# fcogidi/X3D-tf

Hardware: AMD Instinct MI355X
Metric: clips/sec (fwd+bwd) X3D-M 16x224^2; depthwise HBM GB/s (higher is better)
Workload: dtype bf16

## Files before the change

### x3d-tf_amd/csrc/pw_bwd_wst.hip

```cpp
#include <stdlib.h>

#include "pw_gemm_ws.h"

struct PwBwdWstArgs {
  const void* g; const void* yraw; const float* coef;
  const void* wp; int wp_rows;
  void* dx;
  const void* braw; const float* b_ss; const float* egate; double* nc_sums;
  float* dw;
  int N, Co, Ci;
  long long P;
  int tiles_per_block;
  BnBwdFold fold;
  float* slab;
  int hot;
  int noflush;
};

#define BW_YRP 40

template <typename H, int NW, int KS, int CT>
__global__ __launch_bounds__(512, 2) void pw_bwd_wst_kernel(const PwBwdWstArgs a) {
  typedef typename HV<H>::x8 hx8;
  extern __shared__ __attribute__((aligned(16))) unsigned char smem_raw[];
  typedef H T;
  constexpr int BN = 32, OP = WS_OP, NT = 512, Kp = KS * 16, WP = Kp + 8, CoP = CT * 32, YRP = BW_YRP;
  static_assert(CoP >= Kp, "the row-read copy covers every staged dY row");
  constexpr int NSV = (Kp * 4 + NT - 1) / NT;
  H* Yt = (H*)smem_raw;
  H* Yr = (H*)(smem_raw + (size_t)2 * Kp * 64);
  H* Xh = (H*)(smem_raw + (size_t)2 * Kp * 64 + (size_t)2 * CoP * YRP * 2);
  float* Cs = (float*)(smem_raw + (size_t)2 * Kp * 64 + (size_t)2 * CoP * YRP * 2 + (size_t)NW * 32 * YRP * 2);
  float* Os = Cs + Kp * 4;
  const int tid = threadIdx.x, lane = tid & 63, wid = tid >> 6;
  const int r = lane & 31, half = lane >> 5;
  const int mt = (a.Ci + 31) >> 5;
  const int tiles_per_n = (int)((a.P + BN - 1) / BN);
  const int total_tiles = tiles_per_n * a.N;
  const int tile_begin = blockIdx.x * a.tiles_per_block;
  const int tile_end = min(tile_begin + a.tiles_per_block, total_tiles);
  if (tile_begin >= tile_end) return;
  float* myOs = Os + wid * 32 * OP;
  const int rb = blockIdx.y * NW + wid;
  const bool mw = wid < NW && rb < mt;

  {
    hx8 z;
#pragma unroll
    for (int e = 0; e < 8; e++) z[e] = (H)0.f;
    for (int i = tid; i < 2 * CoP * YRP / 8; i += NT) ((hx8*)Yr)[i] = z;
    for (int k = tid; k < Kp; k += NT) {
      f32x4 c = {0.f, 0.f, 0.f, 0.f};
      if (k < a.Co) {
        float cA_, cB_, cC_;
        bn_bwd_coef_load(a.coef, a.fold, k, blockIdx.x == 0 && blockIdx.y == 0, cA_, cB_, cC_);
        c[0] = cA_; c[1] = cB_; c[2] = cC_;
      }
      *(f32x4*)&Cs[k * 4] = c;
    }
  }

  hx8 A[KS];
  if (mw) {
    const H* wt = (const H*)a.wp + (long long)a.wp_rows * WP + ((long long)rb * KS * 64 + lane) * 8;
#pragma unroll
    for (int ks = 0; ks < KS; ks++) A[ks] = *(const hx8*)(wt + ks * 512);
  } else {
#pragma unroll
    for (int ks = 0; ks < KS; ks++)
#pragma unroll
      for (int e = 0; e < 8; e++) A[ks][e] = (H)0.f;
  }

  hx8 g0[NSV], y0[NSV], g1[NSV], y1[NSV];
  auto issue_loads = [&](int tile_, hx8 (&gr)[NSV], hx8 (&yr)[NSV]) {
    const int tile = a.hot ? tile_begin : min(tile_, tile_end - 1);
    const int n = tile / tiles_per_n;
    const long long p0 = (long long)(tile - n * tiles_per_n) * BN;
#pragma unroll
    for (int i = 0; i < NSV; i++) {
      const int v = tid + i * NT;
      const int k = v >> 2;
      const long long p = p0 + (v & 3) * 8;
      const bool ok = k < a.Co && p < a.P;
      const long long o = ok ? ((long long)n * a.Co + k) * a.P + p : 0;
      gr[i] = *(const hx8*)((const T*)a.g + o);
      yr[i] = *(const hx8*)((const T*)a.yraw + o);
    }
  };
  auto commit = [&](int tile, int buf, const hx8 (&gr)[NSV], const hx8 (&yr)[NSV]) {
    const int n = tile / tiles_per_n;
    const long long p0 = (long long)(tile - n * tiles_per_n) * BN;
#pragma unroll
    for (int i = 0; i < NSV; i++) {
      const int v = tid + i * NT;
      const int k = v >> 2;
      if (k >= Kp) continue;
      const bool ok = k < a.Co && p0 + (v & 3) * 8 < a.P;
      const f32x4 cf = *(const f32x4*)&Cs[k * 4];
      float val[8];
#pragma unroll
      for (int e = 0; e < 8; e++) val[e] = ok ? cf[0] * (float)gr[i][e] + cf[1] * (float)yr[i][e] + cf[2] : 0.f;
      hx8 hv;
#pragma unroll
      for (int e = 0; e < 8; e++) hv[e] = (H)val[e];
      *(hx8*)&Yt[(buf * Kp + k) * BN + (v & 3) * 8] = hv;
      *(hx8*)&Yr[(buf * CoP + k) * YRP + (v & 3) * 8] = hv;
    }
  };

  const int row = lane >> 1, c0 = 16 * (lane & 1);
  const int m = rb * 32 + row;
  const bool mrow = mw && m < a.Ci;
  hx8 eb0[2], eb1[2];
  float gl0, gl1;
  const float* gsrc = a.egate ? a.egate : a.b_ss;
  auto issue_braw = [&](int tile_, hx8 (&eb)[2], float& gl) {
    const int tile = a.hot ? tile_begin : min(tile_, tile_end - 1);
    const int n = tile / tiles_per_n;
    const long long p0 = (long long)(tile - n * tiles_per_n) * BN;
    gl = gsrc[(a.egate && mrow) ? (long long)n * a.Ci + m : 0];
#pragma unroll
    for (int hv = 0; hv < 2; hv++) {
      const long long p = p0 + c0 + 8 * hv;
      const long long o = (mrow && p < a.P) ? ((long long)n * a.Ci + m) * a.P + p : 0;
      eb[hv] = *(const hx8*)((const T*)a.braw + o);
    }
  };

  float st1 = 0.f, st2 = 0.f;
  auto flush_sums = [&](int n) {
    const float s1 = st1 + dpp_get<0xB1, 0xF>(st1), s2 = st2 + dpp_get<0xB1, 0xF>(st2);
    if (mrow && (lane & 1) == 0) {
      double* d = a.nc_sums + ((long long)n * a.Ci + m) * 2;
      atomic_add_d(d, (double)s1);
      atomic_add_d(d + 1, (double)s2);
    }
    st1 = 0.f;
    st2 = 0.f;
  };
  const float sb = mrow ? a.b_ss[m * 2] : 0.f, tb = mrow ? a.b_ss[m * 2 + 1] : 0.f;

  f32x16 acc_dw[CT];
#pragma unroll
  for (int s = 0; s < CT; s++)
#pragma unroll
    for (int e = 0; e < 16; e++) acc_dw[s][e] = 0.f;

  const int g16 = lane >> 4, q = (lane & 15) >> 2, pp = lane & 3;
  const int tr_off = (8 * (g16 >> 1) + q) * BN + 16 * (g16 & 1) + 4 * pp;
  typedef s16x4 __attribute__((address_space(3))) * lds_s16x4_ptr;

  int n_prev = tile_begin / tiles_per_n;
  issue_loads(tile_begin, g0, y0);
  issue_braw(tile_begin, eb0, gl0);
  __syncthreads();
  commit(tile_begin, 0, g0, y0);
  __syncthreads();
  issue_loads(tile_begin + 1, g1, y1);
  issue_loads(tile_begin + 2, g0, y0);

  typedef __attribute__((ext_vector_type(4))) unsigned int u32x4_;
  auto step = [&](int tile, int cur, hx8 (&gr)[NSV], hx8 (&yr)[NSV], hx8 (&eb)[2], float gl, hx8 (&ebn)[2], float& gln) {
    const int n = tile / tiles_per_n;
    const long long p0 = (long long)(tile - n * tiles_per_n) * BN;
    if (n != n_prev) flush_sums(n_prev);
    n_prev = n;
    issue_braw(tile + 1, ebn, gln);
    const float gt = (mrow && a.egate) ? gl : 1.0f;
    __amdgpu_buffer_rsrc_t dxr = __builtin_amdgcn_make_buffer_rsrc((T*)a.dx + (long long)n * a.Ci * a.P, 0,
                                                                   (int)((long long)a.Ci * a.P * 2), 0x00020000);

    f32x16 acc;
#pragma unroll
    for (int e = 0; e < 16; e++) acc[e] = 0.f;
    if (mw) {
      const H* xb = Yt + cur * (Kp * BN) + tr_off;
#pragma unroll
      for (int ks = 0; ks < KS; ks++) {
        const s16x4 b0 = __builtin_amdgcn_ds_read_tr16_b64_v4i16((lds_s16x4_ptr)(xb + ks * 16 * BN));
        const s16x4 b1 = __builtin_amdgcn_ds_read_tr16_b64_v4i16((lds_s16x4_ptr)(xb + (ks * 16 + 4) * BN));
        const s16x8 bs = {b0[0], b0[1], b0[2], b0[3], b1[0], b1[1], b1[2], b1[3]};
        acc = mfma16<H>(A[ks], __builtin_bit_cast(hx8, bs), acc);
      }
    }

    if (tile + 1 < tile_end) commit(tile + 1, cur ^ 1, gr, yr);

    if (mw) {
#pragma unroll
      for (int e = 0; e < 16; e++) myOs[((e & 3) + 8 * (e >> 2) + 4 * half) * OP + r] = acc[e];
#pragma unroll
      for (int hv = 0; hv < 2; hv++) {
        const long long p = p0 + c0 + 8 * hv;
        const bool ok = mrow && p < a.P;
        float val[8];
        {
          const f32x4 v0 = *(const f32x4*)&myOs[row * OP + c0 + 8 * hv], v1 = *(const f32x4*)&myOs[row * OP + c0 + 8 * hv + 4];
#pragma unroll
          for (int e = 0; e < 4; e++) { val[e] = v0[e]; val[4 + e] = v1[e]; }
        }
        hx8 xh;
        const SwishCoef sc_ = swish_coef(sb, tb, gt);
#pragma unroll
        for (int e = 0; e < 8; e++) {
          const float b = (float)eb[hv][e];
          float xs, d_;
          swish_bwd_(sc_, b, xs, d_);
          xh[e] = ok ? (H)xs : (H)0.f;
          const float dv = val[e] * d_;
          val[e] = dv;
          if (ok) { st1 += dv; st2 += dv * b; }
        }
        *(hx8*)&Xh[(wid * 32 + row) * YRP + c0 + 8 * hv] = xh;
        hx8 ov;
#pragma unroll
        for (int e = 0; e < 8; e++) ov[e] = (H)val[e];
        __builtin_amdgcn_raw_buffer_store_b128(__builtin_bit_cast(u32x4_, ov), dxr,
                                               ok ? (unsigned)(((long long)m * a.P + p) * 2) : 0x80000000u, 0, 0);
      }
      const H* yrow = Yr + (cur * CoP + r) * YRP + 8 * half;
      const H* xrow = Xh + (wid * 32 + r) * YRP + 8 * half;
#pragma unroll
      for (int ks = 0; ks < BN / 16; ks++) {
        const hx8 bf = *(const hx8*)(xrow + ks * 16);
#pragma unroll
        for (int s = 0; s < CT; s++) {
          const hx8 af = *(const hx8*)(yrow + s * 32 * YRP + ks * 16);
          acc_dw[s] = mfma16<H>(af, bf, acc_dw[s]);
        }
      }
    }
    __syncthreads();
    issue_loads(tile + 3, gr, yr);
  };
  for (int tile = tile_begin; tile < tile_end; tile += 2) {
    step(tile, 0, g1, y1, eb0, gl0, eb1, gl1);
    if (tile + 1 < tile_end) step(tile + 1, 1, g0, y0, eb1, gl1, eb0, gl0);
  }
  flush_sums(n_prev);

  if (mw && !a.noflush) {
    const int ci = rb * 32 + r;
    float* slab = a.slab ? a.slab + (long long)blockIdx.x * a.Co * a.Ci : nullptr;
#pragma unroll
    for (int s = 0; s < CT; s++)
#pragma unroll
      for (int e = 0; e < 16; e++) {
        const int co = s * 32 + (e & 3) + 8 * (e >> 2) + 4 * half;
        if (co < a.Co && ci < a.Ci) {
          if (slab) slab[(long long)co * a.Ci + ci] = acc_dw[s][e];
          else atomicAdd(&a.dw[(long long)co * a.Ci + ci], acc_dw[s][e]);
        }
      }
  }
}

template <int NW, int KS, int CT>
static inline size_t bw_lds_bytes() {
  return (size_t)2 * KS * 16 * 64 + (size_t)2 * CT * 32 * BW_YRP * 2 + (size_t)NW * 32 * BW_YRP * 2 + (size_t)KS * 16 * 16 +
         (size_t)NW * 32 * WS_OP * 4;
}

bool pw_bwd_wst_applies(const x3d_pw_bwd_args* b) {
  if (x3d_env_int("X3D_PW_BWD_WST", 1) == 0) return false;
  if (!x3d_is_half(b->dtype) || !b->w_panel || (!b->coef && !b->coef_fold) || !b->yraw || b->epi != X3D_EPI_SWISH_BWD || b->tail_c) return false;
  const int ks = (b->Cout + 15) >> 4;
  if (!((b->Cin > 128 && b->Cin <= 224 && ks == 6) || (b->Cin > 224 && b->Cin <= 448 && ks == 12 && x3d_env_int("X3D_PW_BWD_WST5", 1) != 0))) return false;
  const long long P = (long long)b->T * b->H * b->W;
  if (P % 8 || P >= (1ll << 31) || (long long)b->Cin * P * 2 >= (1ll << 31)) return false;
  const void* ps[] = {b->g, b->yraw, b->dx, b->w_panel, b->braw};
  for (const void* p : ps) if (!p || ((uintptr_t)p % 16)) return false;
  return true;
}

static inline void bw_grid(int N, long long P, int Ci, long long* tpb, long long* gx, int* slices) {
  *slices = ceil_div(ceil_div(Ci, 32), 7);
  x3d_persistent_grid(ceil_div_ll(P, 32) * N, x3d_device_cus() / *slices, tpb, gx);
}

template <typename H, int KS, int CT>
static int bw_launch(PwBwdWstArgs& a, hipStream_t st) {
  constexpr int NW = 7;
  const size_t lds = bw_lds_bytes<NW, KS, CT>();
  X3D_DESCRIBE("pw_bwd_wst_kernel<%s, %d, %d, %d>", HV<H>::name, NW, KS, CT);
  auto kern = pw_bwd_wst_kernel<H, NW, KS, CT>;
  static bool attr_set = false;
  if (!attr_set) {
    (void)hipFuncSetAttribute((const void*)kern, hipFuncAttributeMaxDynamicSharedMemorySize, 128 * 1024);
    attr_set = true;
  }
  const long long total_tiles = ceil_div_ll(a.P, 32) * a.N;
  X3D_REQUIRE(total_tiles < (1ll << 31), "pw_bwd_wst: too many tiles");
  long long tpb, gx;
  int slices;
  bw_grid(a.N, a.P, a.Ci, &tpb, &gx, &slices);
  a.tiles_per_block = (int)tpb;
  a.noflush = x3d_env_int("X3D_PW_BWD_NOFLUSH", 0);
  a.hot = x3d_env_int("X3D_PW_BWD_HOT", 0);
  hipLaunchKernelGGL(kern, dim3((unsigned)gx, (unsigned)slices), dim3(512), lds, st, a);
  X3D_LAUNCH_CHECK("pw_bwd_wst");
  return X3D_OK;
}

int pw_bwd_wst(const x3d_pw_bwd_args* b, hipStream_t st) {
  X3D_REQUIRE(b->braw && b->b_scale_shift && b->nc_sums, "pw_bwd: SWISH_BWD needs braw/b_scale_shift/nc_sums");
  PwBwdWstArgs a;
  memset(&a, 0, sizeof(a));
  a.g = b->g; a.yraw = b->yraw; a.coef = b->coef;
  a.wp = b->w_panel; a.wp_rows = (b->Cin + 31) & ~31;
  a.dx = b->dx; a.braw = b->braw; a.b_ss = b->b_scale_shift; a.egate = b->gate; a.nc_sums = b->nc_sums;
  a.dw = b->dw; a.slab = b->dw_slab; a.fold = bn_bwd_fold_arg(b->coef_fold);
  a.N = b->N; a.Co = b->Cout; a.Ci = b->Cin;
  a.P = (long long)b->T * b->H * b->W;
// ... 11 lines not shown
```

### x3d-tf_amd/csrc/dw_mx.hip

```cpp
#include "dw_common.h"

#define MX_PITCH 48
#define MX_ROWS 18
#define MX_TILE (MX_PITCH * MX_ROWS)

struct DwMxFwdArgs {
  DwFwdArgs f;
  unsigned bytes;
};

template <typename T> struct MxOp;
template <> struct MxOp<bf16> {
  typedef bf16x8 x8;
  static __device__ __forceinline__ f32x4 mfma(x8 a, x8 b, f32x4 c) { return __builtin_amdgcn_mfma_f32_16x16x32_bf16(a, b, c, 0, 0, 0); }
};
template <> struct MxOp<f16> {
  typedef f16x8 x8;
  static __device__ __forceinline__ f32x4 mfma(x8 a, x8 b, f32x4 c) { return __builtin_amdgcn_mfma_f32_16x16x32_f16(a, b, c, 0, 0, 0); }
};

template <typename T, bool FLIP>
__device__ __forceinline__ void mx_weight_operands(const float* __restrict__ wc, int lane, typename MxOp<T>::x8 (&A)[6]) {
  const int w = lane & 15, g = lane >> 4;
  float wr[27];
// ... 170 lines not shown
    if (lane == 0) {
      if (a.stats) {
        double* sp = stats_replica(a.stats, g.C, (unsigned)blockIdx.x);
        atomic_add_d(&sp[c * 2], (double)q1);
        atomic_add_d(&sp[c * 2 + 1], (double)q2);
      }
      if (a.pool) {
        if constexpr (P7) {
          const int n0 = (int)(blockIdx.x / g.C) * 4;
#pragma unroll
          for (int k = 0; k < 4; k++) if (n0 + k < g.N) atomic_add_d(&a.pool[(long long)(n0 + k) * g.C + c], (double)qp[k]);
        } else {
          atomic_add_d(&a.pool[(long long)mp.n * g.C + c], (double)q1);
        }
      }
    }
  }
}

static bool mx_plane_ok(const DwGeom& g, bool* p7) {
  *p7 = g.H == 7 && g.W == 7;
  return *p7 || (g.H >= 12 && g.H <= 14 && g.W >= 12 && g.W <= 14 && (g.W & 1) == 0);
}

bool dw_fwd_mx_launch(const DwFwdArgs& a, int dtype, int S, hipStream_t st) {
  const DwGeom& g = a.g;
  const int e = x3d_env_int("X3D_DW_MX", 1);
  bool p7;
  if (e == 0 || dtype == X3D_F32 || S != 1 || !mx_plane_ok(g, &p7) || a.bn.stats) return false;
  const long long bytes = (long long)g.N * g.C * g.T * g.H * g.W * 2;
  if (bytes >= (1ll << 30) || (long long)g.C * g.N >= (1ll << 31)) return false;
  if (((uintptr_t)a.x & 3) || ((uintptr_t)a.y & 3)) return false;
  const bool exact = g.T % 4 == 0;
  if (x3d_describe.out) {
    snprintf(x3d_describe.out, x3d_describe.cap, "dw3d_fwd_mx14_kernel<%s, %s, %d>", dtype == X3D_BF16 ? "bf16" : "f16",
             exact ? "4, 4, 4, 1" : "6, 3, 3, 0", (int)p7);
    return true;
  }
  DwMxFwdArgs pa;
  pa.f = a;
  pa.bytes = (unsigned)bytes;
  const dim3 grid((unsigned)(g.C * (p7 ? ceil_div(g.N, 4) : g.N)));
#define MX_FWD(TT, P7_)                                                                                             \
  do {                                                                                                              \
    if (exact) hipLaunchKernelGGL((dw3d_fwd_mx14_kernel<TT, 4, 4, 4, true, P7_>), grid, dim3(64), 0, st, pa);       \
    else hipLaunchKernelGGL((dw3d_fwd_mx14_kernel<TT, 6, 3, 3, false, P7_>), grid, dim3(64), 0, st, pa);            \
  } while (0)
  if (dtype == X3D_BF16) { if (p7) MX_FWD(bf16, true); else MX_FWD(bf16, false); }
  else { if (p7) MX_FWD(f16, true); else MX_FWD(f16, false); }
#undef MX_FWD
  return true;
}

#define MXA_PITCH 80
#define MXA_TILE (MXA_PITCH * MX_ROWS)

struct DwMxBwdArgs {
  DwBwdArgs b;
  unsigned bytes;
};

template <typename T, int UN, int RB, int PD, bool EXACT, bool P7>
__global__ __launch_bounds__(64, 3) void dw3d_bwd_mx14_kernel(const DwMxBwdArgs pa) {
  static_assert(UN % RB == 0 && UN % 2 == 0 && UN % PD == 0, "ring periods RB (dB planes), 2 (A planes) and PD (planes in flight)");
  typedef typename MxOp<T>::x8 x8;
  typedef __attribute__((ext_vector_type(4))) unsigned int u32x4_;
  __shared__ __attribute__((aligned(16))) unsigned char lds[RB * MX_TILE + 2 * MXA_TILE + 64];
  unsigned char* ldsA = lds + RB * MX_TILE;
  const DwBwdArgs& a = pa.b;
  const DwGeom& g = a.g;
  const int lane = threadIdx.x;
  const int h = lane & 15, s = lane >> 4;
  int c;
  MxMap<P7> mp;
  mp.build(lane, blockIdx.x, g.N, g.C, g.T, g.H, g.W, c);

  for (int i = lane; i < (RB * MX_TILE + 2 * MXA_TILE + 64) / 16; i += 64) ((uint4*)lds)[i] = make_uint4(0u, 0u, 0u, 0u);

  x8 Wt[6];
  mx_weight_operands<T, true>(a.w + c * 27, lane, Wt);
  const float sc = a.ss_a[c * 2], sh = a.ss_a[c * 2 + 1];
  float cA = 0.f, cB = 0.f, cC = 0.f;
  if (mp.n < g.N) {
    const float* cf = a.coef_nc + ((long long)mp.n * g.C + c) * 4;
    cA = cf[0]; cB = cf[1]; cC = cf[2];
  }
  const int planeB = mp.planeB;
  const __amdgpu_buffer_rsrc_t rsA = __builtin_amdgcn_make_buffer_rsrc((T*)a.araw, 0, pa.bytes, 0x00020000);
  const __amdgpu_buffer_rsrc_t rsD = __builtin_amdgcn_make_buffer_rsrc((T*)a.dv, 0, pa.bytes, 0x00020000);
  const __amdgpu_buffer_rsrc_t rsR = __builtin_amdgcn_make_buffer_rsrc((T*)a.braw, 0, pa.bytes, 0x00020000);
  const __amdgpu_buffer_rsrc_t rsG = __builtin_amdgcn_make_buffer_rsrc((T*)a.ga, 0, pa.bytes, 0x00020000);
  unsigned char* stgB = lds + (h + 1) * MX_PITCH + s * 8;
  const unsigned char* rd01 = lds + (h + (s >> 1)) * MX_PITCH + (s & 1) * 16;
  const unsigned char* rd2 = lds + (h + 2) * MX_PITCH + (s & 1) * 16;
  const bool lowk = s < 2;
  const unsigned char* rdM = lowk ? lds + (h + 1) * MX_PITCH + (s & 1) * 16 : lds + RB * MX_TILE + 2 * MXA_TILE;
  const int rdM_tile = lowk ? MX_TILE : 0;
  unsigned char* stgA = ldsA + (h + 1) * MXA_PITCH + 16 + s * 8;
  const unsigned char* rdN = ldsA + (h + 1) * MXA_PITCH + 16 + (s & 1) * 16;

  struct Slot { Raw A, D, R; };
  Slot slot[PD];
  auto issue = [&](int t, Slot& q) {
    const int soff = t < g.T ? t * planeB : DW_OOB;
    raw_bload<8>(q.A, rsA, mp.voffL, soff);
    raw_bload<8>(q.D, rsD, mp.voffL, soff);
    raw_bload<8>(q.R, rsR, mp.voffL, soff);
  };
  const unsigned mk0 = mp.mk0, mk1 = mp.mk1;
  auto stage = [&](const Slot& q, int qb, int qa, bool plane_ok) {
    const Raw rA = mp.aligned(q.A), rD = mp.aligned(q.D), rR = mp.aligned(q.R);
    float av[4], bv[4];
#pragma unroll
    for (int e = 0; e < 4; e++) {
      av[e] = fmaxf(__builtin_fmaf(sc, raw_get<T>(rA, e), sh), 0.f);
      bv[e] = __builtin_fmaf(cA, raw_get<T>(rD, e), __builtin_fmaf(cB, raw_get<T>(rR, e), cC));
    }
    const unsigned pm = plane_ok ? 0xffffffffu : 0u;
    const unsigned m0 = mk0 & pm, m1 = mk1 & pm;
    *(uint2*)(stgA + qa * MXA_TILE) = make_uint2(Dot2<T>::pk(av[0], av[1]) & m0, Dot2<T>::pk(av[2], av[3]) & m1);
    *(uint2*)(stgB + qb * MX_TILE) = make_uint2(Dot2<T>::pk(bv[0], bv[1]) & m0, Dot2<T>::pk(bv[2], bv[3]) & m1);
  };

  f32x4 Cw[9];
#pragma unroll
  for (int k = 0; k < 9; k++) Cw[k] = (f32x4){0.f, 0.f, 0.f, 0.f};
  float s1 = 0.f, s2 = 0.f;
  Raw own;

  auto dummy_stores = [&]() { mp.store(rsG, 0u, 0u, DW_OOB); };
#pragma unroll
  for (int p = 0; p < PD; p++) { issue(p, slot[p]); dummy_stores(); }
  stage(slot[0], 1, 0, true);
  own = mp.aligned(slot[0].A);
  issue(PD, slot[0]);
  dummy_stores();

  for (int t0 = 0; t0 < g.T; t0 += UN) {
#pragma unroll
    for (int d = 0; d < UN; d++) {
      const int t = t0 + d;
      if (!EXACT && t >= g.T) break;
      const int qs[3] = {d % RB, (d + 1) % RB, (d + 2) % RB};
      const int sl = (d + 1) % PD;
      stage(slot[sl], qs[2], (d + 1) & 1, t + 1 < g.T);
      const Raw own_next = mp.aligned(slot[sl].A);
      issue(t + 1 + PD, slot[sl]);
      f32x4 acc = {0.f, 0.f, 0.f, 0.f}, acc2 = {0.f, 0.f, 0.f, 0.f};
#pragma unroll
      for (int kt = 0; kt < 3; kt++) {
        const x8 b01 = *(const x8*)(rd01 + qs[kt] * MX_TILE);
        const x8 b2 = *(const x8*)(rd2 + qs[kt] * MX_TILE);
        acc = MxOp<T>::mfma(Wt[2 * kt], b01, acc);
        acc2 = MxOp<T>::mfma(Wt[2 * kt + 1], b2, acc2);
      }
      {
        const unsigned char* pn = rdN + (d & 1) * MXA_TILE;
        const u32x4_ mid = *(const u32x4_*)pn;
        const unsigned prv = *(const unsigned*)(pn - 4), nxt = *(const unsigned*)(pn + 16);
        const unsigned m01 = __builtin_amdgcn_alignbit(mid[1], mid[0], 16), m12 = __builtin_amdgcn_alignbit(mid[2], mid[1], 16),
                       m23 = __builtin_amdgcn_alignbit(mid[3], mid[2], 16);
        const u32x4_ lft = {__builtin_amdgcn_alignbit(mid[0], prv, 16), m01, m12, m23};
        const u32x4_ rgt = {m01, m12, m23, __builtin_amdgcn_alignbit(nxt, mid[3], 16)};
        const x8 n0 = __builtin_bit_cast(x8, lft), n1 = __builtin_bit_cast(x8, mid), n2 = __builtin_bit_cast(x8, rgt);
#pragma unroll
        for (int kt = 0; kt < 3; kt++) {
          const x8 m = *(const x8*)(rdM + qs[2 - kt] * rdM_tile);
          Cw[kt * 3 + 0] = MxOp<T>::mfma(m, n0, Cw[kt * 3 + 0]);
          Cw[kt * 3 + 1] = MxOp<T>::mfma(m, n1, Cw[kt * 3 + 1]);
          Cw[kt * 3 + 2] = MxOp<T>::mfma(m, n2, Cw[kt * 3 + 2]);
          }
      }
      acc += acc2;
      float o4[4];
#pragma unroll
      for (int e = 0; e < 4; e++) {
        const float av = raw_get<T>(own, e);
        o4[e] = (__builtin_fmaf(sc, av, sh) > 0.f && ((e < 2 ? mk0 : mk1) >> (16 * (e & 1)) & 1u)) ? acc[e] : 0.f;
        s1 += o4[e];
        s2 += o4[e] * av;
      }
      mp.store(rsG, Dot2<T>::pk(o4[0], o4[1]), Dot2<T>::pk(o4[2], o4[3]), t * planeB);
      own = own_next;
    }
  }

  float red[29];
#pragma unroll
  for (int kt = 0; kt < 3; kt++)
#pragma unroll
    for (int kw = 0; kw < 3; kw++) {
      float p[3] = {0.f, 0.f, 0.f};
#pragma unroll
      for (int r = 0; r < 4; r++) {
        const int kh = h - (4 * s + r) + 1;
        const float v = Cw[kt * 3 + kw][r];
        p[0] += kh == 0 ? v : 0.f;
        p[1] += kh == 1 ? v : 0.f;
        p[2] += kh == 2 ? v : 0.f;
      }
#pragma unroll
      for (int kh = 0; kh < 3; kh++) red[kt * 9 + kh * 3 + kw] = wave_sum_lane63(p[kh]);
    }
  red[27] = wave_sum_lane63(s1);
  red[28] = wave_sum_lane63(s2);
  dw_flush_sums29(red, lane, a.dw + c * 27, a.a_sums + c * 2);
}

bool dw_bwd_mx_launch(const DwBwdArgs& a, int dtype, int S, hipStream_t st) {
  const DwGeom& g = a.g;
  const int e = x3d_env_int("X3D_DW_MX", 1);
  bool p7;
  if (e == 0 || (dtype != X3D_BF16 && (dtype != X3D_F16 || x3d_env_int("X3D_DW_MX_F16", 1) == 0)) || S != 1 || !mx_plane_ok(g, &p7)) return false;
  if (p7 && e != 7) return false;
  const long long bytes = (long long)g.N * g.C * g.T * g.H * g.W * 2;
  if (bytes >= (1ll << 30) || (long long)g.C * g.N >= (1ll << 31)) return false;
  if (((uintptr_t)a.araw & 3) || ((uintptr_t)a.ga & 3) || ((uintptr_t)a.dv & 3) || ((uintptr_t)a.braw & 3)) return false;
  const bool exact = g.T % 4 == 0 && !(p7 && dtype != X3D_BF16);
  if (x3d_describe.out) {
    snprintf(x3d_describe.out, x3d_describe.cap, "dw3d_bwd_mx14_kernel<%s, %s, %d>", dtype == X3D_BF16 ? "bf16" : "f16", exact ? "4, 4, 2, 1" : "6, 3, 3, 0", (int)p7);
    return true;
  }
  DwMxBwdArgs pa;
  pa.b = a;
  pa.bytes = (unsigned)bytes;
  const dim3 grid((unsigned)(g.C * (p7 ? ceil_div(g.N, 4) : g.N)));
#define MX14_BWD(T_)                                                                                              \
  do {                                                                                                            \
    if (p7) {                                                                                                     \
      if (exact) hipLaunchKernelGGL((dw3d_bwd_mx14_kernel<T_, 4, 4, 2, true, true>), grid, dim3(64), 0, st, pa);    \
      else hipLaunchKernelGGL((dw3d_bwd_mx14_kernel<T_, 6, 3, 3, false, true>), grid, dim3(64), 0, st, pa);         \
    } else {                                                                                                      \
      if (exact) hipLaunchKernelGGL((dw3d_bwd_mx14_kernel<T_, 4, 4, 2, true, false>), grid, dim3(64), 0, st, pa);   \
      else hipLaunchKernelGGL((dw3d_bwd_mx14_kernel<T_, 6, 3, 3, false, false>), grid, dim3(64), 0, st, pa);        \
    }                                                                                                             \
  } while (0)
  if (dtype == X3D_BF16) MX14_BWD(bf16); else MX14_BWD(f16);
#undef MX14_BWD
  return true;
}


#define MXW_PITCH 112
#define MXW_TILE (MXW_PITCH * MX_ROWS)

struct DwMxwBwdArgs {
  DwBwdArgs b;
  unsigned bytes;
  int HT;
};

template <typename T, int UN, int RB, int PD, bool EXACT>
__global__ __launch_bounds__(64, 2) void dw3d_bwd_mxw_kernel(const DwMxwBwdArgs pa) {
  static_assert(UN % RB == 0 && UN % 2 == 0 && UN % PD == 0, "ring periods RB (dB planes), 2 (A planes) and PD (planes in flight)");
  typedef typename MxOp<T>::x8 x8;
  typedef __attribute__((ext_vector_type(4))) unsigned int u32x4_;
  __shared__ __attribute__((aligned(16))) unsigned char lds[(RB + 2) * MXW_TILE + 128];
  unsigned char* ldsA = lds + RB * MXW_TILE;
  const DwBwdArgs& a = pa.b;
  const DwGeom& g = a.g;
  const int lane = threadIdx.x;
  const int n16 = lane & 15, s = lane >> 4;
  const int ht = __builtin_amdgcn_readfirstlane(blockIdx.x % pa.HT);
  const int nc = __builtin_amdgcn_readfirstlane(blockIdx.x / pa.HT);
  const int c = nc % g.C, n = nc / g.C;
  const int H = g.H, W = g.W;
  const int r0 = ht * 14;

  for (int i = lane; i < ((RB + 2) * MXW_TILE + 128) / 16; i += 64) ((uint4*)lds)[i] = make_uint4(0u, 0u, 0u, 0u);

  x8 Wt[9];
  {
    const float* wc = a.w + c * 27;
#pragma unroll
    for (int i = 0; i < 9; i++) {
      const int kt = i / 3, kh = i % 3;
      const float* w3 = wc + (2 - kt) * 9 + (2 - kh) * 3;
      const float w0 = w3[2], w1 = w3[1], w2 = w3[0];
      x8 op;
#pragma unroll
      for (int j = 0; j < 8; j++) {
        const int kw = 8 * s + j - n16 - 7;
        op[j] = (T)(kw == 0 ? w0 : (kw == 1 ? w1 : (kw == 2 ? w2 : 0.f)));
      }
      Wt[i] = op;
    }
  }
  const float sc = a.ss_a[c * 2], sh = a.ss_a[c * 2 + 1];
  const float* cf = a.coef_nc + ((long long)n * g.C + c) * 4;
  const float cA = cf[0], cB = cf[1], cC = cf[2];

  const int planeB = H * W * 2;
  const __amdgpu_buffer_rsrc_t rsA = __builtin_amdgcn_make_buffer_rsrc((T*)a.araw, 0, pa.bytes, 0x00020000);
  const __amdgpu_buffer_rsrc_t rsD = __builtin_amdgcn_make_buffer_rsrc((T*)a.dv, 0, pa.bytes, 0x00020000);
  const __amdgpu_buffer_rsrc_t rsR = __builtin_amdgcn_make_buffer_rsrc((T*)a.braw, 0, pa.bytes, 0x00020000);
  const __amdgpu_buffer_rsrc_t rsG = __builtin_amdgcn_make_buffer_rsrc((T*)a.ga, 0, pa.bytes, 0x00020000);
  const int row = r0 - 1 + n16;
  const bool row_in = row >= 0 && row < H;
  const bool row_own = n16 >= 1 && n16 <= 14 && row < H;
  const long long base = ((long long)n * g.C + c) * g.T * H * W + (long long)row * W;
  int vld[2], vs0[2], vs1[2];
  unsigned mk0[2], mk1[2], eo0[2], eo1[2];
#pragma unroll
  for (int j = 0; j < 2; j++) {
    const int col = 16 * j + 4 * s;
    const bool c0 = col < W, c1 = col + 2 < W;
    vld[j] = (row_in && c0) ? (int)((base + col) * 2) : DW_OOB;
    mk0[j] = (row_in && c0) ? 0xffffffffu : 0u;
    mk1[j] = (row_in && c1) ? 0xffffffffu : 0u;
    eo0[j] = (row_own && c0) ? 1u : 0u;
    eo1[j] = (row_own && c1) ? 1u : 0u;
    vs0[j] = eo0[j] ? (int)((base + col) * 2) : DW_OOB;
    vs1[j] = eo1[j] ? (int)((base + col + 2) * 2) : DW_OOB;
  }
  unsigned char* stgB = lds + (n16 + 1) * MXW_PITCH + 16 + s * 8;
  unsigned char* stgA = ldsA + (n16 + 1) * MXW_PITCH + 16 + s * 8;
  const unsigned char* rdB = lds + n16 * MXW_PITCH + s * 16;
  const unsigned char* rdM = row_own ? lds + (n16 + 1) * MXW_PITCH + 16 + s * 16 : lds + (RB + 2) * MXW_TILE;
  const int rdM_tile = row_own ? MXW_TILE : 0;
  const unsigned char* rdN = ldsA + (n16 + 1) * MXW_PITCH + 16 + s * 16;

  struct Slot { Raw A[2], D[2], R[2]; };
  Slot slot[PD];
  auto issue = [&](int t, Slot& q) {
    const int soff = t < g.T ? t * planeB : DW_OOB;
#pragma unroll
    for (int j = 0; j < 2; j++) {
      raw_bload<8>(q.A[j], rsA, vld[j], soff);
      raw_bload<8>(q.D[j], rsD, vld[j], soff);
      raw_bload<8>(q.R[j], rsR, vld[j], soff);
    }
  };
  auto stage = [&](const Slot& q, int qb, int qa, bool plane_ok) {
    const unsigned pm = plane_ok ? 0xffffffffu : 0u;
#pragma unroll
    for (int j = 0; j < 2; j++) {
      float av[4], bv[4];
#pragma unroll
      for (int e = 0; e < 4; e++) {
        av[e] = fmaxf(__builtin_fmaf(sc, raw_get<T>(q.A[j], e), sh), 0.f);
        bv[e] = __builtin_fmaf(cA, raw_get<T>(q.D[j], e), __builtin_fmaf(cB, raw_get<T>(q.R[j], e), cC));
      }
      const unsigned m0 = mk0[j] & pm, m1 = mk1[j] & pm;
      *(uint2*)(stgA + qa * MXW_TILE + 32 * j) = make_uint2(Dot2<T>::pk(av[0], av[1]) & m0, Dot2<T>::pk(av[2], av[3]) & m1);
      *(uint2*)(stgB + qb * MXW_TILE + 32 * j) = make_uint2(Dot2<T>::pk(bv[0], bv[1]) & m0, Dot2<T>::pk(bv[2], bv[3]) & m1);
    }
  };
  auto store4 = [&](int j, unsigned p0, unsigned p1, int soff) {
    Raw o, o1;
    o.w[0] = p0; o1.w[0] = p1;
    raw_bstore<4>(o, rsG, vs0[j], soff);
    raw_bstore<4>(o1, rsG, vs1[j], soff);
  };
  auto dummy_stores = [&]() { store4(0, 0u, 0u, DW_OOB); store4(1, 0u, 0u, DW_OOB); };

  f32x4 Cw[9];
#pragma unroll
  for (int k = 0; k < 9; k++) Cw[k] = (f32x4){0.f, 0.f, 0.f, 0.f};
  float s1 = 0.f, s2 = 0.f;
  Raw own[2];

#pragma unroll
  for (int p = 0; p < PD; p++) { issue(p, slot[p]); dummy_stores(); }
  stage(slot[0], 1, 0, true);
  own[0] = slot[0].A[0]; own[1] = slot[0].A[1];
  issue(PD, slot[0]);
  dummy_stores();

  for (int t0 = 0; t0 < g.T; t0 += UN) {
#pragma unroll
    for (int d = 0; d < UN; d++) {
      const int t = t0 + d;
      if (!EXACT && t >= g.T) break;
      const int qs[3] = {d % RB, (d + 1) % RB, (d + 2) % RB};
      const int sl = (d + 1) % PD;
      stage(slot[sl], qs[2], (d + 1) & 1, t + 1 < g.T);
      const Raw on0 = slot[sl].A[0], on1 = slot[sl].A[1];
      issue(t + 1 + PD, slot[sl]);
      {
        const unsigned char* pn = rdN + (d & 1) * MXW_TILE;
        const u32x4_ mid = *(const u32x4_*)pn;
        const unsigned prv = *(const unsigned*)(pn - 4), nxt = *(const unsigned*)(pn + 16);
        const unsigned m01 = __builtin_amdgcn_alignbit(mid[1], mid[0], 16), m12 = __builtin_amdgcn_alignbit(mid[2], mid[1], 16),
                       m23 = __builtin_amdgcn_alignbit(mid[3], mid[2], 16);
        const u32x4_ lft = {__builtin_amdgcn_alignbit(mid[0], prv, 16), m01, m12, m23};
        const u32x4_ rgt = {m01, m12, m23, __builtin_amdgcn_alignbit(nxt, mid[3], 16)};
        const x8 n0 = __builtin_bit_cast(x8, lft), n1 = __builtin_bit_cast(x8, mid), n2 = __builtin_bit_cast(x8, rgt);
#pragma unroll
        for (int kt = 0; kt < 3; kt++) {
          const x8 m = *(const x8*)(rdM + qs[2 - kt] * rdM_tile);
          Cw[kt * 3 + 0] = MxOp<T>::mfma(m, n0, Cw[kt * 3 + 0]);
          Cw[kt * 3 + 1] = MxOp<T>::mfma(m, n1, Cw[kt * 3 + 1]);
          Cw[kt * 3 + 2] = MxOp<T>::mfma(m, n2, Cw[kt * 3 + 2]);
        }
      }
#pragma unroll
      for (int j = 0; j < 2; j++) {
        f32x4 acc = {0.f, 0.f, 0.f, 0.f}, acc2 = {0.f, 0.f, 0.f, 0.f}, acc3 = {0.f, 0.f, 0.f, 0.f};
#pragma unroll
        for (int kt = 0; kt < 3; kt++) {
          const unsigned char* pb = rdB + qs[kt] * MXW_TILE + 32 * j;
          acc = MxOp<T>::mfma(Wt[kt * 3 + 0], *(const x8*)(pb), acc);
          acc2 = MxOp<T>::mfma(Wt[kt * 3 + 1], *(const x8*)(pb + MXW_PITCH), acc2);
          acc3 = MxOp<T>::mfma(Wt[kt * 3 + 2], *(const x8*)(pb + 2 * MXW_PITCH), acc3);
        }
        acc += acc2 + acc3;
        float o4[4];
#pragma unroll
        for (int e = 0; e < 4; e++) {
          const float av = raw_get<T>(own[j], e);
          o4[e] = (__builtin_fmaf(sc, av, sh) > 0.f && (e < 2 ? eo0[j] : eo1[j])) ? acc[e] : 0.f;
          s1 += o4[e];
          s2 += o4[e] * av;
        }
        store4(j, Dot2<T>::pk(o4[0], o4[1]), Dot2<T>::pk(o4[2], o4[3]), t * planeB);
      }
      own[0] = on0; own[1] = on1;
    }
  }

  float red[29];
#pragma unroll
  for (int kt = 0; kt < 3; kt++)
#pragma unroll
    for (int kw = 0; kw < 3; kw++) {
      float p[3] = {0.f, 0.f, 0.f};
#pragma unroll
      for (int r = 0; r < 4; r++) {
        const int kh = n16 - (4 * s + r) + 1;
        const float v = Cw[kt * 3 + kw][r];
        p[0] += kh == 0 ? v : 0.f;
        p[1] += kh == 1 ? v : 0.f;
        p[2] += kh == 2 ? v : 0.f;
      }
#pragma unroll
      for (int kh = 0; kh < 3; kh++) red[kt * 9 + kh * 3 + kw] = wave_sum_lane63(p[kh]);
    }
  red[27] = wave_sum_lane63(s1);
  red[28] = wave_sum_lane63(s2);
  dw_flush_sums29(red, lane, a.dw + c * 27, a.a_sums + c * 2);
}

bool dw_bwd_mxw_launch(const DwBwdArgs& a, int dtype, int S, hipStream_t st) {
  const DwGeom& g = a.g;
  const int e = x3d_env_int("X3D_DW_MXW", 1);
  if (e == 0 || (dtype != X3D_BF16 && (dtype != X3D_F16 || x3d_env_int("X3D_DW_MX_F16", 1) == 0)) || S != 1 || (g.W & 1) || g.W < 26 || g.W > 30 || g.H < 12 ||
      (g.H % 14 != 0 && g.H % 14 < 10)) return false;
  const long long bytes = (long long)g.N * g.C * g.T * g.H * g.W * 2;
  const int HT = ceil_div(g.H, 14);
  if (bytes >= (1ll << 30) || (long long)g.C * g.N * HT >= (1ll << 31)) return false;
  if (((uintptr_t)a.araw & 7) || ((uintptr_t)a.ga & 3) || ((uintptr_t)a.dv & 7) || ((uintptr_t)a.braw & 7)) return false;
  const bool exact = g.T % 4 == 0 && dtype == X3D_BF16;
  if (x3d_describe.out) {
    snprintf(x3d_describe.out, x3d_describe.cap, "dw3d_bwd_mxw_kernel<%s, %s>", dtype == X3D_BF16 ? "bf16" : "f16", exact ? "4, 4, 2, 1" : "6, 3, 3, 0");
    return true;
  }
  DwMxwBwdArgs pa;
  pa.b = a;
  pa.bytes = (unsigned)bytes;
  pa.HT = HT;
  const dim3 grid((unsigned)((long long)g.C * g.N * HT));
  if (dtype == X3D_BF16) {
    if (exact) hipLaunchKernelGGL((dw3d_bwd_mxw_kernel<bf16, 4, 4, 2, true>), grid, dim3(64), 0, st, pa);
    else hipLaunchKernelGGL((dw3d_bwd_mxw_kernel<bf16, 6, 3, 3, false>), grid, dim3(64), 0, st, pa);
  } else {
    if (exact) hipLaunchKernelGGL((dw3d_bwd_mxw_kernel<f16, 4, 4, 2, true>), grid, dim3(64), 0, st, pa);
    else hipLaunchKernelGGL((dw3d_bwd_mxw_kernel<f16, 6, 3, 3, false>), grid, dim3(64), 0, st, pa);
  }
  return true;
}
```

Measured before the change: 3256.

## Keep dX GEMM accumulators in registers by swapping MFMA operands, drop LDS staging

Swaps the A/B operands of the dX MFMA and permutes the transpose-read offsets so each lane's accumulator already holds its own output row and column slice. This removes the LDS round-trip through the Os scratch and the Xh buffer, and feeds the swish-backward result straight into the dW MFMA as the B operand. It cuts LDS traffic and LDS footprint, which may allow higher occupancy, and changes the row/column ownership and the cross-lane partial-sum reduction from a DPP to a shuffle. The risk is correctness of the new lane-to-element mapping.

```diff
diff --git a/x3d-tf_amd/csrc/pw_bwd_wst.hip b/x3d-tf_amd/csrc/pw_bwd_wst.hip
--- a/x3d-tf_amd/csrc/pw_bwd_wst.hip
+++ b/x3d-tf_amd/csrc/pw_bwd_wst.hip
@@ -24,14 +24,12 @@
   typedef typename HV<H>::x8 hx8;
   extern __shared__ __attribute__((aligned(16))) unsigned char smem_raw[];
   typedef H T;
-  constexpr int BN = 32, OP = WS_OP, NT = 512, Kp = KS * 16, WP = Kp + 8, CoP = CT * 32, YRP = BW_YRP;
+  constexpr int BN = 32, NT = 512, Kp = KS * 16, WP = Kp + 8, CoP = CT * 32, YRP = BW_YRP;
   static_assert(CoP >= Kp, "the row-read copy covers every staged dY row");
   constexpr int NSV = (Kp * 4 + NT - 1) / NT;
   H* Yt = (H*)smem_raw;
   H* Yr = (H*)(smem_raw + (size_t)2 * Kp * 64);
-  H* Xh = (H*)(smem_raw + (size_t)2 * Kp * 64 + (size_t)2 * CoP * YRP * 2);
-  float* Cs = (float*)(smem_raw + (size_t)2 * Kp * 64 + (size_t)2 * CoP * YRP * 2 + (size_t)NW * 32 * YRP * 2);
-  float* Os = Cs + Kp * 4;
+  float* Cs = (float*)(smem_raw + (size_t)2 * Kp * 64 + (size_t)2 * CoP * YRP * 2);
   const int tid = threadIdx.x, lane = tid & 63, wid = tid >> 6;
   const int r = lane & 31, half = lane >> 5;
   const int mt = (a.Ci + 31) >> 5;
@@ -40,7 +38,6 @@
   const int tile_begin = blockIdx.x * a.tiles_per_block;
   const int tile_end = min(tile_begin + a.tiles_per_block, total_tiles);
   if (tile_begin >= tile_end) return;
-  float* myOs = Os + wid * 32 * OP;
   const int rb = blockIdx.y * NW + wid;
   const bool mw = wid < NW && rb < mt;
 
@@ -109,8 +106,8 @@
     }
   };
 
-  const int row = lane >> 1, c0 = 16 * (lane & 1);
-  const int m = rb * 32 + row;
+  const int c0 = 8 * half;
+  const int m = rb * 32 + r;
   const bool mrow = mw && m < a.Ci;
   hx8 eb0[2], eb1[2];
   float gl0, gl1;
@@ -122,7 +119,7 @@
     gl = gsrc[(a.egate && mrow) ? (long long)n * a.Ci + m : 0];
 #pragma unroll
     for (int hv = 0; hv < 2; hv++) {
-      const long long p = p0 + c0 + 8 * hv;
+      const long long p = p0 + c0 + 16 * hv;
       const long long o = (mrow && p < a.P) ? ((long long)n * a.Ci + m) * a.P + p : 0;
       eb[hv] = *(const hx8*)((const T*)a.braw + o);
     }
@@ -130,8 +127,8 @@
 
   float st1 = 0.f, st2 = 0.f;
   auto flush_sums = [&](int n) {
-    const float s1 = st1 + dpp_get<0xB1, 0xF>(st1), s2 = st2 + dpp_get<0xB1, 0xF>(st2);
-    if (mrow && (lane & 1) == 0) {
+    const float s1 = st1 + __shfl_xor(st1, 32, 64), s2 = st2 + __shfl_xor(st2, 32, 64);
+    if (mrow && half == 0) {
       double* d = a.nc_sums + ((long long)n * a.Ci + m) * 2;
       atomic_add_d(d, (double)s1);
       atomic_add_d(d + 1, (double)s2);
@@ -148,7 +145,7 @@
     for (int e = 0; e < 16; e++) acc_dw[s][e] = 0.f;
 
   const int g16 = lane >> 4, q = (lane & 15) >> 2, pp = lane & 3;
-  const int tr_off = (8 * (g16 >> 1) + q) * BN + 16 * (g16 & 1) + 4 * pp;
+  const int tr_off = (8 * (g16 >> 1) + q) * BN + 16 * (g16 & 1) + 4 * (((pp & 1) << 1) | (pp >> 1));
   typedef s16x4 __attribute__((address_space(3))) * lds_s16x4_ptr;
 
   int n_prev = tile_begin / tiles_per_n;
@@ -181,53 +178,36 @@
         const s16x4 b0 = __builtin_amdgcn_ds_read_tr16_b64_v4i16((lds_s16x4_ptr)(xb + ks * 16 * BN));
         const s16x4 b1 = __builtin_amdgcn_ds_read_tr16_b64_v4i16((lds_s16x4_ptr)(xb + (ks * 16 + 4) * BN));
         const s16x8 bs = {b0[0], b0[1], b0[2], b0[3], b1[0], b1[1], b1[2], b1[3]};
-        acc = mfma16<H>(A[ks], __builtin_bit_cast(hx8, bs), acc);
+        acc = mfma16<H>(__builtin_bit_cast(hx8, bs), A[ks], acc);
       }
     }
 
     if (tile + 1 < tile_end) commit(tile + 1, cur ^ 1, gr, yr);
 
     if (mw) {
-#pragma unroll
-      for (int e = 0; e < 16; e++) myOs[((e & 3) + 8 * (e >> 2) + 4 * half) * OP + r] = acc[e];
+      const SwishCoef sc_ = swish_coef(sb, tb, gt);
+      const H* yrow = Yr + (cur * CoP + r) * YRP + 8 * half;
 #pragma unroll
       for (int hv = 0; hv < 2; hv++) {
-        const long long p = p0 + c0 + 8 * hv;
+        const long long p = p0 + c0 + 16 * hv;
         const bool ok = mrow && p < a.P;
-        float val[8];
-        {
-          const f32x4 v0 = *(const f32x4*)&myOs[row * OP + c0 + 8 * hv], v1 = *(const f32x4*)&myOs[row * OP + c0 + 8 * hv + 4];
-#pragma unroll
-          for (int e = 0; e < 4; e++) { val[e] = v0[e]; val[4 + e] = v1[e]; }
-        }
-        hx8 xh;
-        const SwishCoef sc_ = swish_coef(sb, tb, gt);
+        hx8 xh, ov;
 #pragma unroll
         for (int e = 0; e < 8; e++) {
           const float b = (float)eb[hv][e];
           float xs, d_;
           swish_bwd_(sc_, b, xs, d_);
           xh[e] = ok ? (H)xs : (H)0.f;
-          const float dv = val[e] * d_;
-          val[e] = dv;
+          const float dv = acc[8 * hv + e] * d_;
+          ov[e] = (H)dv;
           if (ok) { st1 += dv; st2 += dv * b; }
         }
-        *(hx8*)&Xh[(wid * 32 + row) * YRP + c0 + 8 * hv] = xh;
-        hx8 ov;
-#pragma unroll
-        for (int e = 0; e < 8; e++) ov[e] = (H)val[e];
         __builtin_amdgcn_raw_buffer_store_b128(__builtin_bit_cast(u32x4_, ov), dxr,
                                                ok ? (unsigned)(((long long)m * a.P + p) * 2) : 0x80000000u, 0, 0);
-      }
-      const H* yrow = Yr + (cur * CoP + r) * YRP + 8 * half;
-      const H* xrow = Xh + (wid * 32 + r) * YRP + 8 * half;
-#pragma unroll
-      for (int ks = 0; ks < BN / 16; ks++) {
-        const hx8 bf = *(const hx8*)(xrow + ks * 16);
 #pragma unroll
         for (int s = 0; s < CT; s++) {
-          const hx8 af = *(const hx8*)(yrow + s * 32 * YRP + ks * 16);
-          acc_dw[s] = mfma16<H>(af, bf, acc_dw[s]);
+          const hx8 af = *(const hx8*)(yrow + s * 32 * YRP + hv * 16);
+          acc_dw[s] = mfma16<H>(af, xh, acc_dw[s]);
         }
       }
     }
@@ -258,8 +238,7 @@
 
 template <int NW, int KS, int CT>
 static inline size_t bw_lds_bytes() {
-  return (size_t)2 * KS * 16 * 64 + (size_t)2 * CT * 32 * BW_YRP * 2 + (size_t)NW * 32 * BW_YRP * 2 + (size_t)KS * 16 * 16 +
-         (size_t)NW * 32 * WS_OP * 4;
+  return (size_t)2 * KS * 16 * 64 + (size_t)2 * CT * 32 * BW_YRP * 2 + (size_t)KS * 16 * 16;
 }
 
 bool pw_bwd_wst_applies(const x3d_pw_bwd_args* b) {
```

After: 3249. No clear change (-0.2%).

## Cut register pressure in depthwise backward MFMA kernels and raise wave occupancy

Applied to the files above, without the earlier changes.

Uniform per-channel scalars are moved into SGPRs with readfirstlane, and the channel and batch indices are pinned as scalars. The lane id is recomputed at the end of the kernel instead of being kept live. Per-lane 32-bit masks and store offsets become booleans, with the store offset derived from the load offset. The wide backward kernel's launch bounds rise to 3 waves for exact bf16. Sched barriers and asm pins limit compiler reordering, which risks spills or lost latency hiding in exchange for the lower VGPR count and higher occupancy.

```diff
diff --git a/x3d-tf_amd/csrc/dw_mx.hip b/x3d-tf_amd/csrc/dw_mx.hip
--- a/x3d-tf_amd/csrc/dw_mx.hip
+++ b/x3d-tf_amd/csrc/dw_mx.hip
@@ -246,6 +246,16 @@
   return true;
 }
 
+__device__ __forceinline__ void mx_pin_sgpr(int& v) { asm volatile("" : "+s"(v)); }
+__device__ __forceinline__ float mx_uniform(float v) { return __builtin_bit_cast(float, __builtin_amdgcn_readfirstlane(__builtin_bit_cast(int, v))); }
+template <typename T> __device__ __forceinline__ typename MxOp<T>::x8 mx_pin_operand(typename MxOp<T>::x8 op) {
+  typedef __attribute__((ext_vector_type(4))) unsigned int u4_;
+  u4_ pin = __builtin_bit_cast(u4_, op);
+  asm volatile("" : "+v"(pin));
+  return __builtin_bit_cast(typename MxOp<T>::x8, pin);
+}
+__device__ __forceinline__ int mx_lane_again() { return (int)__builtin_amdgcn_mbcnt_hi(~0u, __builtin_amdgcn_mbcnt_lo(~0u, 0u)); }
+
 #define MXA_PITCH 80
 #define MXA_TILE (MXA_PITCH * MX_ROWS)
 
@@ -268,17 +278,21 @@
   int c;
   MxMap<P7> mp;
   mp.build(lane, blockIdx.x, g.N, g.C, g.T, g.H, g.W, c);
+  mx_pin_sgpr(c);
 
   for (int i = lane; i < (RB * MX_TILE + 2 * MXA_TILE + 64) / 16; i += 64) ((uint4*)lds)[i] = make_uint4(0u, 0u, 0u, 0u);
 
   x8 Wt[6];
   mx_weight_operands<T, true>(a.w + c * 27, lane, Wt);
-  const float sc = a.ss_a[c * 2], sh = a.ss_a[c * 2 + 1];
+#pragma unroll
+  for (int i = 0; i < 6; i++) Wt[i] = mx_pin_operand<T>(Wt[i]);
+  const float sc = mx_uniform(a.ss_a[c * 2]), sh = mx_uniform(a.ss_a[c * 2 + 1]);
   float cA = 0.f, cB = 0.f, cC = 0.f;
   if (mp.n < g.N) {
     const float* cf = a.coef_nc + ((long long)mp.n * g.C + c) * 4;
     cA = cf[0]; cB = cf[1]; cC = cf[2];
   }
+  if constexpr (!P7) { cA = mx_uniform(cA); cB = mx_uniform(cB); cC = mx_uniform(cC); }
   const int planeB = mp.planeB;
   const __amdgpu_buffer_rsrc_t rsA = __builtin_amdgcn_make_buffer_rsrc((T*)a.araw, 0, pa.bytes, 0x00020000);
   const __amdgpu_buffer_rsrc_t rsD = __builtin_amdgcn_make_buffer_rsrc((T*)a.dv, 0, pa.bytes, 0x00020000);
@@ -288,8 +302,8 @@
   const unsigned char* rd01 = lds + (h + (s >> 1)) * MX_PITCH + (s & 1) * 16;
   const unsigned char* rd2 = lds + (h + 2) * MX_PITCH + (s & 1) * 16;
   const bool lowk = s < 2;
-  const unsigned char* rdM = lowk ? lds + (h + 1) * MX_PITCH + (s & 1) * 16 : lds + RB * MX_TILE + 2 * MXA_TILE;
-  const int rdM_tile = lowk ? MX_TILE : 0;
+  const unsigned char* rdM = lds + (lowk ? (h + 1) * MX_PITCH : 0) + (s & 1) * 16;
+  constexpr int rdM_tile = MX_TILE;
   unsigned char* stgA = ldsA + (h + 1) * MXA_PITCH + 16 + s * 8;
   const unsigned char* rdN = ldsA + (h + 1) * MXA_PITCH + 16 + (s & 1) * 16;
 
@@ -302,6 +316,7 @@
     raw_bload<8>(q.R, rsR, mp.voffL, soff);
   };
   const unsigned mk0 = mp.mk0, mk1 = mp.mk1;
+  const bool ok0 = mp.mk0 != 0u, ok1 = mp.mk1 != 0u;
   auto stage = [&](const Slot& q, int qb, int qa, bool plane_ok) {
     const Raw rA = mp.aligned(q.A), rD = mp.aligned(q.D), rR = mp.aligned(q.R);
     float av[4], bv[4];
@@ -310,10 +325,16 @@
       av[e] = fmaxf(__builtin_fmaf(sc, raw_get<T>(rA, e), sh), 0.f);
       bv[e] = __builtin_fmaf(cA, raw_get<T>(rD, e), __builtin_fmaf(cB, raw_get<T>(rR, e), cC));
     }
-    const unsigned pm = plane_ok ? 0xffffffffu : 0u;
-    const unsigned m0 = mk0 & pm, m1 = mk1 & pm;
-    *(uint2*)(stgA + qa * MXA_TILE) = make_uint2(Dot2<T>::pk(av[0], av[1]) & m0, Dot2<T>::pk(av[2], av[3]) & m1);
-    *(uint2*)(stgB + qb * MX_TILE) = make_uint2(Dot2<T>::pk(bv[0], bv[1]) & m0, Dot2<T>::pk(bv[2], bv[3]) & m1);
+    if constexpr (P7) {
+      const unsigned pm = plane_ok ? 0xffffffffu : 0u;
+      const unsigned m0 = mk0 & pm, m1 = mk1 & pm;
+      *(uint2*)(stgA + qa * MXA_TILE) = make_uint2(Dot2<T>::pk(av[0], av[1]) & m0, Dot2<T>::pk(av[2], av[3]) & m1);
+      *(uint2*)(stgB + qb * MX_TILE) = make_uint2(Dot2<T>::pk(bv[0], bv[1]) & m0, Dot2<T>::pk(bv[2], bv[3]) & m1);
+    } else {
+      const bool m0 = ok0 && plane_ok, m1 = ok1 && plane_ok;
+      *(uint2*)(stgA + qa * MXA_TILE) = make_uint2(m0 ? Dot2<T>::pk(av[0], av[1]) : 0u, m1 ? Dot2<T>::pk(av[2], av[3]) : 0u);
+      *(uint2*)(stgB + qb * MX_TILE) = make_uint2(m0 ? Dot2<T>::pk(bv[0], bv[1]) : 0u, m1 ? Dot2<T>::pk(bv[2], bv[3]) : 0u);
+    }
   };
 
   f32x4 Cw[9];
@@ -365,20 +386,33 @@
           Cw[kt * 3 + 2] = MxOp<T>::mfma(m, n2, Cw[kt * 3 + 2]);
           }
       }
+      __builtin_amdgcn_sched_barrier(0);
       acc += acc2;
       float o4[4];
 #pragma unroll
       for (int e = 0; e < 4; e++) {
         const float av = raw_get<T>(own, e);
-        o4[e] = (__builtin_fmaf(sc, av, sh) > 0.f && ((e < 2 ? mk0 : mk1) >> (16 * (e & 1)) & 1u)) ? acc[e] : 0.f;
+        const bool in = P7 ? (((e < 2 ? mk0 : mk1) >> (16 * (e & 1)) & 1u) != 0u) : (e < 2 ? ok0 : ok1);
+        o4[e] = (__builtin_fmaf(sc, av, sh) > 0.f && in) ? acc[e] : 0.f;
         s1 += o4[e];
         s2 += o4[e] * av;
       }
-      mp.store(rsG, Dot2<T>::pk(o4[0], o4[1]), Dot2<T>::pk(o4[2], o4[3]), t * planeB);
+      if constexpr (P7) {
+        mp.store(rsG, Dot2<T>::pk(o4[0], o4[1]), Dot2<T>::pk(o4[2], o4[3]), t * planeB);
+      } else {
+        Raw o, o1;
+        o.w[0] = Dot2<T>::pk(o4[0], o4[1]); o1.w[0] = Dot2<T>::pk(o4[2], o4[3]);
+        int v = mp.voffL;
+        asm volatile("" : "+v"(v));
+        raw_bstore<4>(o, rsG, v, t * planeB);
+        raw_bstore<4>(o1, rsG, (ok1 ? v : DW_OOB) + 4, t * planeB);
+      }
       own = own_next;
-    }
-  }
-
+      if constexpr (!P7) __builtin_amdgcn_sched_barrier(0);
+    }
+  }
+
+  const int lane_e = mx_lane_again();
   float red[29];
 #pragma unroll
   for (int kt = 0; kt < 3; kt++)
@@ -387,7 +421,7 @@
       float p[3] = {0.f, 0.f, 0.f};
 #pragma unroll
       for (int r = 0; r < 4; r++) {
-        const int kh = h - (4 * s + r) + 1;
+        const int kh = (lane_e & 15) - (4 * (lane_e >> 4) + r) + 1;
         const float v = Cw[kt * 3 + kw][r];
         p[0] += kh == 0 ? v : 0.f;
         p[1] += kh == 1 ? v : 0.f;
@@ -398,7 +432,7 @@
     }
   red[27] = wave_sum_lane63(s1);
   red[28] = wave_sum_lane63(s2);
-  dw_flush_sums29(red, lane, a.dw + c * 27, a.a_sums + c * 2);
+  dw_flush_sums29(red, lane_e, a.dw + c * 27, a.a_sums + c * 2);
 }
 
 bool dw_bwd_mx_launch(const DwBwdArgs& a, int dtype, int S, hipStream_t st) {
@@ -438,6 +472,8 @@
 #define MXW_PITCH 112
 #define MXW_TILE (MXW_PITCH * MX_ROWS)
 
+#define MXW_WAVES(T, EXACT) (((EXACT) && __is_same(T, bf16)) ? 3 : 2)
+
 struct DwMxwBwdArgs {
   DwBwdArgs b;
   unsigned bytes;
@@ -445,7 +481,7 @@
 };
 
 template <typename T, int UN, int RB, int PD, bool EXACT>
-__global__ __launch_bounds__(64, 2) void dw3d_bwd_mxw_kernel(const DwMxwBwdArgs pa) {
+__global__ __launch_bounds__(64, MXW_WAVES(T, EXACT)) void dw3d_bwd_mxw_kernel(const DwMxwBwdArgs pa) {
   static_assert(UN % RB == 0 && UN % 2 == 0 && UN % PD == 0, "ring periods RB (dB planes), 2 (A planes) and PD (planes in flight)");
   typedef typename MxOp<T>::x8 x8;
   typedef __attribute__((ext_vector_type(4))) unsigned int u32x4_;
@@ -457,7 +493,9 @@
   const int n16 = lane & 15, s = lane >> 4;
   const int ht = __builtin_amdgcn_readfirstlane(blockIdx.x % pa.HT);
   const int nc = __builtin_amdgcn_readfirstlane(blockIdx.x / pa.HT);
-  const int c = nc % g.C, n = nc / g.C;
+  int c = nc % g.C, n = nc / g.C;
+  mx_pin_sgpr(c);
+  mx_pin_sgpr(n);
   const int H = g.H, W = g.W;
   const int r0 = ht * 14;
 
@@ -477,12 +515,12 @@
         const int kw = 8 * s + j - n16 - 7;
         op[j] = (T)(kw == 0 ? w0 : (kw == 1 ? w1 : (kw == 2 ? w2 : 0.f)));
       }
-      Wt[i] = op;
-    }
-  }
-  const float sc = a.ss_a[c * 2], sh = a.ss_a[c * 2 + 1];
+      Wt[i] = mx_pin_operand<T>(op);
+    }
+  }
+  const float sc = mx_uniform(a.ss_a[c * 2]), sh = mx_uniform(a.ss_a[c * 2 + 1]);
   const float* cf = a.coef_nc + ((long long)n * g.C + c) * 4;
-  const float cA = cf[0], cB = cf[1], cC = cf[2];
+  const float cA = mx_uniform(cf[0]), cB = mx_uniform(cf[1]), cC = mx_uniform(cf[2]);
 
   const int planeB = H * W * 2;
   const __amdgpu_buffer_rsrc_t rsA = __builtin_amdgcn_make_buffer_rsrc((T*)a.araw, 0, pa.bytes, 0x00020000);
@@ -493,25 +531,23 @@
   const bool row_in = row >= 0 && row < H;
   const bool row_own = n16 >= 1 && n16 <= 14 && row < H;
   const long long base = ((long long)n * g.C + c) * g.T * H * W + (long long)row * W;
-  int vld[2], vs0[2], vs1[2];
-  unsigned mk0[2], mk1[2], eo0[2], eo1[2];
+  int vld[2];
+  bool mk0[2], mk1[2], eo0[2], eo1[2];
 #pragma unroll
   for (int j = 0; j < 2; j++) {
     const int col = 16 * j + 4 * s;
     const bool c0 = col < W, c1 = col + 2 < W;
     vld[j] = (row_in && c0) ? (int)((base + col) * 2) : DW_OOB;
-    mk0[j] = (row_in && c0) ? 0xffffffffu : 0u;
-    mk1[j] = (row_in && c1) ? 0xffffffffu : 0u;
-    eo0[j] = (row_own && c0) ? 1u : 0u;
-    eo1[j] = (row_own && c1) ? 1u : 0u;
-    vs0[j] = eo0[j] ? (int)((base + col) * 2) : DW_OOB;
-    vs1[j] = eo1[j] ? (int)((base + col + 2) * 2) : DW_OOB;
+    mk0[j] = row_in && c0;
+    mk1[j] = row_in && c1;
+    eo0[j] = row_own && c0;
+    eo1[j] = row_own && c1;
   }
   unsigned char* stgB = lds + (n16 + 1) * MXW_PITCH + 16 + s * 8;
   unsigned char* stgA = ldsA + (n16 + 1) * MXW_PITCH + 16 + s * 8;
   const unsigned char* rdB = lds + n16 * MXW_PITCH + s * 16;
-  const unsigned char* rdM = row_own ? lds + (n16 + 1) * MXW_PITCH + 16 + s * 16 : lds + (RB + 2) * MXW_TILE;
-  const int rdM_tile = row_own ? MXW_TILE : 0;
+  const unsigned char* rdM = lds + (row_own ? (n16 + 1) * MXW_PITCH : 0) + 16 + s * 16;
+  constexpr int rdM_tile = MXW_TILE;
   const unsigned char* rdN = ldsA + (n16 + 1) * MXW_PITCH + 16 + s * 16;
 
   struct Slot { Raw A[2], D[2], R[2]; };
@@ -526,7 +562,6 @@
     }
   };
   auto stage = [&](const Slot& q, int qb, int qa, bool plane_ok) {
-    const unsigned pm = plane_ok ? 0xffffffffu : 0u;
 #pragma unroll
     for (int j = 0; j < 2; j++) {
       float av[4], bv[4];
@@ -535,16 +570,18 @@
         av[e] = fmaxf(__builtin_fmaf(sc, raw_get<T>(q.A[j], e), sh), 0.f);
         bv[e] = __builtin_fmaf(cA, raw_get<T>(q.D[j], e), __builtin_fmaf(cB, raw_get<T>(q.R[j], e), cC));
       }
-      const unsigned m0 = mk0[j] & pm, m1 = mk1[j] & pm;
-      *(uint2*)(stgA + qa * MXW_TILE + 32 * j) = make_uint2(Dot2<T>::pk(av[0], av[1]) & m0, Dot2<T>::pk(av[2], av[3]) & m1);
-      *(uint2*)(stgB + qb * MXW_TILE + 32 * j) = make_uint2(Dot2<T>::pk(bv[0], bv[1]) & m0, Dot2<T>::pk(bv[2], bv[3]) & m1);
+      const bool m0 = mk0[j] && plane_ok, m1 = mk1[j] && plane_ok;
+      *(uint2*)(stgA + qa * MXW_TILE + 32 * j) = make_uint2(m0 ? Dot2<T>::pk(av[0], av[1]) : 0u, m1 ? Dot2<T>::pk(av[2], av[3]) : 0u);
+      *(uint2*)(stgB + qb * MXW_TILE + 32 * j) = make_uint2(m0 ? Dot2<T>::pk(bv[0], bv[1]) : 0u, m1 ? Dot2<T>::pk(bv[2], bv[3]) : 0u);
     }
   };
   auto store4 = [&](int j, unsigned p0, unsigned p1, int soff) {
     Raw o, o1;
     o.w[0] = p0; o1.w[0] = p1;
-    raw_bstore<4>(o, rsG, vs0[j], soff);
-    raw_bstore<4>(o1, rsG, vs1[j], soff);
+    int v = vld[j];
+    asm volatile("" : "+v"(v));
+    raw_bstore<4>(o, rsG, eo0[j] ? v : DW_OOB, soff);
+    raw_bstore<4>(o1, rsG, (eo1[j] ? v : DW_OOB) + 4, soff);
   };
   auto dummy_stores = [&]() { store4(0, 0u, 0u, DW_OOB); store4(1, 0u, 0u, DW_OOB); };
 
@@ -590,6 +627,7 @@
       }
 #pragma unroll
       for (int j = 0; j < 2; j++) {
+        __builtin_amdgcn_sched_barrier(0);
         f32x4 acc = {0.f, 0.f, 0.f, 0.f}, acc2 = {0.f, 0.f, 0.f, 0.f}, acc3 = {0.f, 0.f, 0.f, 0.f};
 #pragma unroll
         for (int kt = 0; kt < 3; kt++) {
@@ -613,6 +651,7 @@
     }
   }
 
+  const int lane_e = mx_lane_again();
   float red[29];
 #pragma unroll
   for (int kt = 0; kt < 3; kt++)
@@ -621,7 +660,7 @@
       float p[3] = {0.f, 0.f, 0.f};
 #pragma unroll
       for (int r = 0; r < 4; r++) {
-        const int kh = n16 - (4 * s + r) + 1;
+        const int kh = (lane_e & 15) - (4 * (lane_e >> 4) + r) + 1;
         const float v = Cw[kt * 3 + kw][r];
         p[0] += kh == 0 ? v : 0.f;
         p[1] += kh == 1 ? v : 0.f;
@@ -632,7 +671,7 @@
     }
   red[27] = wave_sum_lane63(s1);
   red[28] = wave_sum_lane63(s2);
-  dw_flush_sums29(red, lane, a.dw + c * 27, a.a_sums + c * 2);
+  dw_flush_sums29(red, lane_e, a.dw + c * 27, a.a_sums + c * 2);
 }
 
 bool dw_bwd_mxw_launch(const DwBwdArgs& a, int dtype, int S, hipStream_t st) {
```

Result: no change. 3228 before, 3258 after (median of 6 runs) (+0.9%).
